# ShawnHymel/ei-keyword-spotting

Measured on AMD Instinct MI355X. Metric: 1s@16kHz clips/sec (MFCC+CNN), higher is better.
Workload: dtype f32

## Files before the change

### ei-keyword-spotting_amd/csrc/kws_fast.hip

```cpp
#include <atomic>

#include "kws_device.h"
#include "kws_fast.h"
#include "kws_bfly_m2k1.h"
#include "kws_fast_maxmin.h"
#if KWS_FAST_WPS >= 3
#define kws_fast_kernel kws_fast_kernel_w3
#define kws_launch_fast kws_launch_fast_w3
#define kws_launch_fast_prof kws_launch_fast_prof_w3
#endif
#include "kws_nn_int8_dev.h"

typedef float v4f __attribute__((ext_vector_type(4)));
#if KWS_FAST_WPS >= 3
#define KWS_OPAQUE3(v) asm volatile("" : "+v"(v))
#define KWS_LANE3(lane) ((int)__builtin_amdgcn_mbcnt_hi(~0u, __builtin_amdgcn_mbcnt_lo(~0u, 0u)))
#define KWS_FAST_SINK (shared + FP.sink_off)
#else
#define KWS_OPAQUE3(v) do { } while (0)
#define KWS_LANE3(lane) (lane)
#define KWS_FAST_SINK (F + FP.sink_off)
#endif
static_assert(KWS_FAST_ZF == KWS_ZF && KWS_FAST_WAVE == KWS_WAVE, "kws_fast.h mirrors kws_device.h");

template <int CTRL> __device__ __forceinline__ float dpp_mov(float v)
{
    return __int_as_float(__builtin_amdgcn_update_dpp(0, __float_as_int(v), CTRL, 0xf, 0xf, true));
}
__device__ __forceinline__ float half_wave_sum(float v)
{
    v += dpp_mov<0xB1>(v);
    v += dpp_mov<0x4E>(v);
    v += dpp_mov<0x141>(v);
    v += dpp_mov<0x140>(v);
    v += __int_as_float(__builtin_amdgcn_ds_swizzle(__float_as_int(v), 0x401F));
    return v;
}
__device__ __forceinline__ float wave_max(float v)
{
    v = fast_max(v, dpp_mov<0xB1>(v));
    v = fast_max(v, dpp_mov<0x4E>(v));
    v = fast_max(v, dpp_mov<0x141>(v));
    v = fast_max(v, dpp_mov<0x140>(v));
    v = fast_max(v, __int_as_float(__builtin_amdgcn_ds_swizzle(__float_as_int(v), 0x401F)));
    return fast_max(v, __shfl_xor(v, 32, KWS_WAVE));
}
__device__ __forceinline__ float wave_sum(float v)
{
    v = half_wave_sum(v);
    return v + __shfl_xor(v, 32, KWS_WAVE);
}
__device__ __forceinline__ float group_sum(float v, int S)
{
    if (S > 1) v += dpp_mov<0xB1>(v);
    if (S > 2) v += dpp_mov<0x4E>(v);
    if (S > 4) v += dpp_mov<0x141>(v);
// ... 746 lines not shown
        WAVE_SYNC();
        if constexpr (SPLIT) {
            _Float16 *const hcol = (_Float16 *)((char *)img + 4 * cb) + cl;
            const bool col_on = lane_on && c < in_cp;
            _Float16 *dst_i = col_on ? hcol + r0 * (2 * fs) : (_Float16 *)sink;
            const int dst_step = col_on ? 2 * fs : 0;
            float sc = c < ncep ? (float)(1 << KWS_SPLIT22_PRE_EXP) : 0.0f;
#pragma unroll
            for (int i = 0; i < CR; ++i) asm volatile("" : "+v"(o[i]));
#pragma unroll
            for (int i = 0; i < CR; ++i) {
                const bool live = CMVN_ROW_LIVE(r0, i);
                _Float16 hi, lo;
                const float d = kws_split22(o[i], sc, &hi, &lo);
                _Float16 *const dst = live ? dst_i : (_Float16 *)sink;
                dst[0] = hi;
                dst[KWS_FAST_PRE_LO / 2] = lo;
                dst_i += dst_step;
                sc = __fmaf_rn(d, 0.0f, sc);
                vacc = live ? __fmaf_rn(gq[i], gq[i], vacc) : vacc;
            }
            vacc = (SAFE > 0 || r0 < nfr) ? __fmaf_rn(sc, 0.0f, vacc) : vacc;
        } else {
#pragma unroll
        for (int i = 0; i < CR; ++i) {
            const int r = r0 + i;
            const bool live = act && r < nfr;
            *(live ? col + r * fs : sink) = o[i];
            if constexpr (DEFER) vacc = live ? __fmaf_rn(gq[i], gq[i], vacc) : vacc;
        }
        }
    }
    WAVE_SYNC();
    return vacc;
#undef CMVN_ROW_LIVE
#undef CMVN_ROW
}

#define KWS_FAST_NPHASE 20
#ifndef KWS_FAST_FULL_PASS
#define KWS_FAST_FULL_PASS (KWS_FAST_WPS >= 3)
#endif
#ifndef KWS_FAST_SOFS
#define KWS_FAST_SOFS (KWS_FAST_WPS >= 3)
#endif
#ifndef KWS_FAST_LATE_ELOG
#define KWS_FAST_LATE_ELOG (KWS_FAST_WPS >= 3)
#endif
#if KWS_FAST_LATE_ELOG
#define KWS_FAST_ELOG(e) (e)
#else
#define KWS_FAST_ELOG(e) fast_log((e) == 0.0f ? FLT_EPSILON : (e))
#endif
#define FPH(i) do { if (PROF) { const long long now_ = clock64(); ph[i] += now_ - tlast; tlast = now_; } } while (0)

template <int NZ, int DG, bool PROF = false, bool FROM_CEP = false, bool NET = true, int QCP = 0, bool MFE = false>
__global__ __launch_bounds__(256 * KWS_FAST_WPS, KWS_FAST_WPS) void kws_fast_kernel(KwsDspPlan P, const KwsFastPlan *__restrict__ FPp, const int16_t *__restrict__ pcm, int n_clips,
                                                          float *__restrict__ scores, float *__restrict__ features,
                                                          int8_t *__restrict__ q_out, float in_scale, int in_zp,
                                                          int *__restrict__ flag_count, int *__restrict__ flag_list,
                                                          long long *__restrict__ prof_out = nullptr, const float *__restrict__ cep = nullptr,
                                                          const KwsNnPlan *__restrict__ QNp = nullptr, const int *__restrict__ sel = nullptr,
                                                          float *__restrict__ tap_logits = nullptr, int feat_in = 0)
{
    static_assert(QCP == 0 || !NET, "the int8 network follows the feature-emitting form");
    static_assert(!MFE || (!NET && QCP == 0 && !FROM_CEP && !PROF), "the MFE form is the spectral prefix: mel energies to HBM");
    const KwsFastPlan &FP = *FPp;
    extern __shared__ __attribute__((aligned(16))) float lds[];
    const int lane = threadIdx.x & (KWS_WAVE - 1), wave = __builtin_amdgcn_readfirstlane((int)(threadIdx.x >> 6));
    if (FROM_CEP && (int)blockIdx.x * (int)(blockDim.x >> 6) >= sel_count(sel, n_clips)) return;
    float *shared = lds;
    float *F = lds + FP.shared_floats + FP.q_floats + wave * FP.wave_floats;
    float *R1 = F + FP.f_floats;
    float *xw = R1, *pw = R1;
    for (int i = threadIdx.x; i < FP.shared_floats; i += blockDim.x) shared[i] = FP.shared_init[i];
    for (int i = lane; i < FP.r1_floats; i += KWS_WAVE) R1[i] = 0.0f;
    constexpr int Q_HEAD = 48 * 256, Q_WB1 = Q_HEAD + ((KWS_HEAD_BYTES + 15) & ~15), Q_WB2 = Q_WB1 + (QCP == 16 ? 4 : 16) * KWS_WAVE * 16,
                  Q_RQ = Q_WB2 + 4 * KWS_WAVE * 16;
    if constexpr (QCP != 0) {
        unsigned char *const qs = (unsigned char *)(lds + FP.shared_floats);
        const KwsNnPlan &QN = *QNp;
        for (int i = threadIdx.x * 4; i < QN.blk[0].out_c * 256; i += blockDim.x * 4) *(int *)(qs + i) = *(const int *)(QN.blk[0].add_lut + i);
        for (int i = threadIdx.x * 4; i < QN.blk[1].out_c * 256; i += blockDim.x * 4) *(int *)(qs + 32 * 256 + i) = *(const int *)(QN.blk[1].add_lut + i);
        (void)nn_head_stage(QN, qs + Q_HEAD);
        nn_mfma_stage_lds<QCP == 0 ? 16 : QCP>(QN, (v4i *)(qs + Q_WB1), (v4i *)(qs + Q_WB2), (int *)(qs + Q_RQ));
    }
    if constexpr (FROM_CEP)
        for (int i = lane; i < FP.wave_floats; i += KWS_WAVE) F[i] = 0.0f;
    __syncthreads();

    const int nfr = P.n_frames, ncep = P.n_cepstral, NF = 8 * DG;
    const int n_tail = (nfr >= KWS_FAST_MEL_CHUNK && (nfr & 7) != 0 && (nfr & 7) <= 2) ? (nfr & 7) : 0;
    const int n_pass = n_tail ? nfr / KWS_FAST_MEL_CHUNK : (nfr + KWS_FAST_MEL_CHUNK - 1) / KWS_FAST_MEL_CHUNK;
    const int fs = FP.fs;
    float *img = F;
    float *elog = F + nfr * fs;
    constexpr int NZ2 = DG > 4 ? KWS_FAST_NZ2 : 1;
    const float *dct_frag = shared + FP.dct_off;
    const int pstride = FP.pstride;
    const int n_waves = blockDim.x >> 6;
    const float pre_cof = P.pre_cof, pscale = kws_fast_pscale(P.inv_fft);
    const int frame_stride = P.frame_stride, n_samples = P.n_samples;
    const float *cnt_tab = shared + FP.cnt_off;
    const int *upd_tab = (const int *)(shared + FP.upd_off);
    const float *ext_tab = FP.ext_off >= 0 ? shared + FP.ext_off : nullptr;
    const float inv_win = FP.inv_win;
    const float *guard_tab = shared + (FROM_CEP ? FP.guard_cep_off : FP.guard_off);
    const int *pad_idx = (const int *)(shared + FP.pad_off);
    const int win_size = P.win_size, prow = nfr + 2 * P.pad;
    const int cr = FP.cr, n_blocks = FP.n_blocks, n_labels = FP.n_labels;
    (void)cr;
    long long ph[KWS_FAST_NPHASE] = { 0 }, tlast = PROF ? clock64() : 0;

    const int clip_stride = gridDim.x * n_waves;
    float *const stash = F + FP.stash_off;
    bool have_stash = false;
    const int n_sel = FROM_CEP ? sel_count(sel, n_clips) : n_clips;
#if KWS_FAST_WPS >= 3
    static_assert(!FROM_CEP, "the forms that start from cepstra are not built for three waves per SIMD");
    int *const tk = FP.tickets;
    int ni = 0;
    for (int ci = blockIdx.x * n_waves + wave; ci < n_sel; ci = ni) {
        int tv = 0;
        if (KWS_LANE3(lane) == 0) tv = __hip_atomic_fetch_add(tk, 1, __ATOMIC_RELAXED, __HIP_MEMORY_SCOPE_AGENT);
        const int clip = FROM_CEP ? sel_clip(sel, ci) : ci;
        const int next_ci = ci;
#else
    for (int ci = blockIdx.x * n_waves + wave; ci < n_sel; ci += clip_stride) {
        const int clip = FROM_CEP ? sel_clip(sel, ci) : ci;
        const int next_ci = ci + clip_stride;
        const int next_clip = ci + clip_stride < n_sel ? ci + clip_stride : -1;
#endif
        int lane_c = KWS_LANE3(lane);
        asm volatile("" : "+v"(lane_c));
        const int fl = lane_c & 7, fg = lane_c >> 3;
        const int nbA = (fl >> 2) + 4 * (fl & 3);
        const float a_c = P.tw[16].x, a_e = P.tw[32].x;
        const cf b1 = to_cf(P.tw[4 * fl]), b2 = to_cf(P.tw[8 * fl]), b3 = to_cf(P.tw[12 * fl]);
#if KWS_FAST_WPS >= 3
        const float *const twl_c = shared + FP.twl_off + 24 * fl, *const twl_s = shared + FP.twl_off + 192 + 16 * fl;
#else
        cf c1[4], c2[4], c3[4];
    #pragma unroll
        for (int a = 0; a < 4; ++a) { c1[a] = to_cf(P.tw[fl + 8 * a]); c2[a] = to_cf(P.tw[2 * (fl + 8 * a)]); c3[a] = to_cf(P.tw[3 * (fl + 8 * a)]); }
        cf stw[8];
    #pragma unroll
        for (int q = 0; q < 8; ++q) {
            const int k = fl + 8 * (q & 3) + 32 * (q >> 2);
            stw[q] = to_cf(P.stw[(k == 0 ? KWS_NC / 2 : k) - 1]);
        }
#endif
        const int xwr = fg * KWS_FAST_XS + 18 * fl;
        const int xrd = fg * KWS_FAST_XS + 2 * fl;
        const int partner = (lane_c & ~7) | ((8 - fl) & 7);
        const int half = lane_c >> 5, t = lane_c & 31;
        const int start1 = FP.tap_start1[lane_c], start2 = FP.tap_start2[lane_c];
        float lvl_sum = 0.0f;
        float w1[NZ], w2[NZ2];
    #pragma unroll
        for (int n = 0; n < NZ; ++n) w1[n] = FP.tap_w1[lane_c * KWS_FAST_NZ_MAX + n];
    #pragma unroll
        for (int n = 0; n < NZ2; ++n) w2[n] = FP.tap_w2[lane_c * KWS_FAST_NZ2 + n];
        int touched_a = 0, touched_b = 0;
        if constexpr (FROM_CEP) {
            const float *src = cep + (size_t)clip * (nfr * ncep);
            const int n_val = nfr * ncep;
            const unsigned inv = (1u << 20) / (unsigned)ncep + 1u;
            const int rr = P.ring_rows, rh = P.ring_head;
            auto ring = [&](int r) { const int t = r + rh; return (rr != 0 && r < rr) ? (t >= rr ? t - rr : t) : r; };
            auto trips = [&](int i_from, int i_to) {
                for (int i0 = i_from + lane; i0 - lane < i_to; i0 += 4 * KWS_WAVE) {
                    float v[4];
                    int dst[4];
// ... 93 lines not shown
                    macc[s] = MFE ? a : fast_log(a);
                }
                float *const d1 = img + (fbase + 4 * half) * fs + t;
#pragma unroll
                for (int s = 0; s < 4; ++s) d1[s * fs] = macc[s];
                if (DG > 4) img[(fbase + sl2) * fs + j2] = macc[4];
                return;
            }
#pragma unroll
            for (int s2 = 0; s2 < 4; s2 += 2) {
                if (s2 >= 2 * pairs) break;
                float xv[2][NZ];
#pragma unroll
                for (int s = 0; s < 2; ++s)
#pragma unroll
                    for (int n = 0; n < NZ; ++n) xv[s][n] = p1[(s2 + s) * pstride + n];
#pragma unroll
                for (int s = 0; s < 2; ++s) {
                    float acc = 0.0f;
#pragma unroll
                    for (int n = 0; n < NZ; ++n) acc = __fmaf_rn(xv[s][n], w1[n], acc);
                    macc[s2 + s] = acc;
                }
            }
            float acc2 = 0.0f;
            if (DG > 4) {
                float xv2[NZ2];
#pragma unroll
                for (int n = 0; n < NZ2; ++n) xv2[n] = p2[n];
#pragma unroll
                for (int n = 0; n < NZ2; ++n) acc2 = __fmaf_rn(xv2[n], w2[n], acc2);
            }
            macc[4] = acc2;
#pragma unroll
            for (int s = 0; s < 5; ++s) {
                const float a = macc[s] == 0.0f ? FLT_EPSILON : macc[s];
                macc[s] = MFE ? a : fast_log(a);
            }
#pragma unroll
            for (int s = 0; s < 4; ++s) {
                const int slot = 4 * half + s;
                if (slot < nfc && t < NF) img[(fbase + slot) * fs + t + (slot == 1 ? adj1 : 0)] = macc[s];
            }
            if (DG > 4 && sl2 < nfc && j2 < NF) img[(fbase + sl2) * fs + j2 + (sl2 == 1 ? adj1 : 0)] = macc[4];
        };
        fast_i2 nxt[2][8];
#if KWS_FAST_SOFS
        if constexpr (SOFS) fetch_at(std::true_type(), sofs0, nxt);
        else
#endif
        fetch(0, nxt);
        int touched = touch(1);
#if KWS_FAST_WPS >= 3
        ni = clip_stride + __builtin_amdgcn_readfirstlane(tv);
        const int next_clip = ni < n_sel ? ni : -1;
#endif
        const bool pair_tail = n_tail == 1 && !have_stash && next_clip >= 0;
        int touched_tail = 0;
        const int16_t *const xnext = pcm + (size_t)max(next_clip, 0) * n_samples;
        if (pair_tail && lane_c < 8) touched_tail = *(const int *)(xnext + (nfr - 1) * frame_stride + 32 * lane_c);
#if KWS_FAST_WPS >= 3
        auto pass_body = [&](int q) {
#else
        for (int q = 0; q < n_pass; ++q) {
#endif
            const int fbase = KWS_FAST_MEL_CHUNK * q;
            const int f = fbase + fg;
            const bool live = f < nfr;
            cf u[4][4];
            {
                cf z[2][8];
#pragma unroll
                for (int blk = 0; blk < 2; ++blk)
#pragma unroll
                    for (int i = 0; i < 8; ++i) z[blk][i] = fast_point(nxt[blk][i], pre_cof);
                if (f == 0 && fl == 0) {
                    fast_i2 v = nxt[0][0];
                    v.y = v.x;
                    v.x = wrap_prev << 16;
                    z[0][0] = fast_point(v, pre_cof);
                }
                fetch(q + 1, nxt);
                asm volatile("" : : "v"(touched));
                touched = touch(q + 2);
                FPH(0);
#pragma unroll
                for (int blk = 0; blk < 2; ++blk) {
                    cf sm[4], df[4];
#pragma unroll
                    for (int i = 0; i < 4; ++i) { sm[i] = cadd(z[blk][2 * i], z[blk][2 * i + 1]); df[i] = csub(z[blk][2 * i], z[blk][2 * i + 1]); }
                    bfly4_unit(sm[0], sm[1], sm[2], sm[3]);
                    bfly4_m2k1(df[0], df[1], df[2], df[3], a_c, a_e);
#pragma unroll
                    for (int i = 0; i < 4; ++i) { z[blk][2 * i] = sm[i]; z[blk][2 * i + 1] = df[i]; }
                }
#pragma unroll
                for (int rnd = 0; rnd < 2; ++rnd) {
#pragma unroll
                    for (int r = 0; r < 8; ++r) *(float2 *)(xw + xwr + 2 * r) = make_float2(z[rnd][r].r, z[rnd][r].i);
                    WAVE_SYNC();
#pragma unroll
                    for (int b = 0; b < 2; ++b)
#pragma unroll
                        for (int a = 0; a < 4; ++a) {
                            const float2 v = *(const float2 *)(xw + xrd + 18 * a + 72 * b);
                            u[a][2 * rnd + b].r = v.x; u[a][2 * rnd + b].i = v.y;
                        }
                    WAVE_SYNC();
                }
            }
#pragma unroll
            for (int b = 0; b < 4; ++b) bfly4(u[0][b], u[1][b], u[2][b], u[3][b], b1, b2, b3);
#pragma unroll
#if KWS_FAST_WPS >= 3
            for (int a = 0; a < 4; ++a) {
                const float4 c12 = *(const float4 *)(twl_c + 6 * a);
                const float2 c3v = *(const float2 *)(twl_c + 6 * a + 4);
                cf t1, t2, t3;
                t1.r = c12.x; t1.i = c12.y; t2.r = c12.z; t2.i = c12.w; t3.r = c3v.x; t3.i = c3v.y;
                bfly4(u[a][0], u[a][1], u[a][2], u[a][3], t1, t2, t3);
            }
            cf stw[8];
#pragma unroll
            for (int q = 0; q < 8; q += 2) {
                const float4 v = *(const float4 *)(twl_s + 2 * q);
                stw[q].r = v.x; stw[q].i = v.y; stw[q + 1].r = v.z; stw[q + 1].i = v.w;
            }
#else
            for (int a = 0; a < 4; ++a) bfly4(u[a][0], u[a][1], u[a][2], u[a][3], c1[a], c2[a], c3[a]);
#endif
            FPH(1);
            {
                float *prow = pw + fg * pstride;
                const bool lane0 = fl == 0;
                float esum = 0.0f;
#pragma unroll
                for (int qq = 0; qq < 8; ++qq) {
// ... 274 lines not shown
            if constexpr (!FROM_CEP) {
                if (silent && FP.sil_off >= 0) {
                    const int half_nf = min(NF / 2, ncep - 1);
                    const float sv = shared[FP.sil_off + min(lane_m + 1, 31)];
                    float *const dst = img + 1 + lane_m;
                    for (unsigned long long mm = smask; mm != 0ull; mm &= mm - 1ull) {
                        const int r = __builtin_ctzll(mm);
                        if (lane_m < half_nf) dst[r * fs] = sv;
                    }
                    n_silent = __popcll(smask);
                    WAVE_SYNC();
                }
            }
            const float mu = wave_sum(on ? x0 : 0.0f) * FP.c0_inv_rows;
            const float d0 = on ? x0 - mu : 0.0f;
            const float sd0 = __builtin_amdgcn_sqrtf(wave_sum(d0 * d0) * FP.c0_inv_rows);
            const float top = wave_max(on ? fabsf(x0) : 0.0f);
            c0_exact = silent || !(FP.c0_factor * sd0 >= __fmaf_rn(FP.c0_rel, top, FP.c0_abs));
        }
        if (c0_exact) {
            constexpr int PS = 260;
            float *pc = R1;
            for (int p = lane_m; p < prow; p += KWS_WAVE) {
                int prw[4];
                float pvv[4];
#pragma unroll
                for (int sft = 0; sft < 4; ++sft) prw[sft] = pad_idx[min(p + sft, prow - 1)];
#pragma unroll
                for (int sft = 0; sft < 4; ++sft) pvv[sft] = img[prw[sft] * fs];
#pragma unroll
                for (int sft = 0; sft < 4; ++sft) pc[sft * PS + p] = pvv[sft];
            }
            WAVE_SYNC();
            const int r = min(lane_m, nfr - 1);
            const float4 *pv = (const float4 *)(pc + (r & 3) * PS + (r & ~3));
            float sum = 0.0f;
            int q = 0;
            const int nq = win_size >> 2;
            for (; q + 4 <= nq; q += 4) {
                float4 v[4];
#pragma unroll
                for (int e = 0; e < 4; ++e) v[e] = pv[q + e];
#pragma unroll
                for (int e = 0; e < 4; ++e) { sum += v[e].x; sum += v[e].y; sum += v[e].z; sum += v[e].w; }
            }
            for (; q < nq; ++q) { const float4 v = pv[q]; sum += v.x; sum += v.y; sum += v.z; sum += v.w; }
            {
                const float4 v = pv[q];
                const int rem = win_size & 3;
                if (rem > 0) sum += v.x;
                if (rem > 1) sum += v.y;
                if (rem > 2) sum += v.z;
            }
            if (lane_m < nfr) elog[lane_m] = __fdiv_rn(sum, (float)win_size);
            WAVE_SYNC();
        }
        if (PROF) { const long long now_ = clock64(); ph[19] += now_ - tlast; }
        if constexpr (QCP != 0) {
            const int z1 = (int)((unsigned)(QNp->blk[0].in_zp & 0xff) * 0x01010101u);
            for (int i = lane_m; i < KWS_A1_ROWS * (QCP / 4); i += KWS_WAVE) ((int *)act1)[i] = z1;
            WAVE_SYNC();
        }
        float gV = 0.0f;
        if constexpr (!MFE) {
          if (feats_given) gV = FP.v_net_feat;
          else {
            float level = FROM_CEP ? 0.0f : wave_sum(lvl_sum) * FP.lvl_inv, abs_scale = 1.0f;
            if (!FROM_CEP && n_silent > 0) {
                const float live = (float)(nfr - n_silent), rows = (float)nfr;
                level = live > 0.0f ? fmaxf(__fmaf_rn(level, rows, (float)n_silent * fast_log(FLT_EPSILON)), 0.0f) / live : 0.0f;
                abs_scale = __builtin_amdgcn_sqrtf(live / rows);
                level *= abs_scale;
            }
#if KWS_FAST_WPS >= 3
            constexpr bool TWO_COPIES = !(NZ == 8 && DG == 5);
            if (TWO_COPIES && nfr >= 3 * 13 + 9) vlane = fast_cmvn<13, 16, true, true, 9>(img, cnt_tab, upd_tab, fs, inv_win, guard_tab, level, abs_scale, silent, FP.sys_t2, piv_row, elog, c0_exact, lane_m, nfr, ncep, ext_tab, csink, FP.blk[0].in_cp);
            else vlane = fast_cmvn<13, 16, true, true>(img, cnt_tab, upd_tab, fs, inv_win, guard_tab, level, abs_scale, silent, FP.sys_t2, piv_row, elog, c0_exact, lane_m, nfr, ncep, ext_tab, csink, FP.blk[0].in_cp);
#else
            if (cr == 13) vlane = fast_cmvn<13, 16, QCP == 0>(img, cnt_tab, upd_tab, fs, inv_win, guard_tab, level, abs_scale, silent, FP.sys_t2, piv_row, elog, c0_exact, lane_m, nfr, ncep, ext_tab, csink);
            else vlane = fast_cmvn<17, 20, QCP == 0>(img, cnt_tab, upd_tab, fs, inv_win, guard_tab, level, abs_scale, silent, FP.sys_t2, piv_row, elog, c0_exact, lane_m, nfr, ncep, ext_tab, csink);
#endif
            gV = __int_as_float(__builtin_amdgcn_readfirstlane(__float_as_int(wave_sum(vlane) + FP.v_net)));
          }
        }
        if constexpr (!NET) {
            if (!MFE && !(gV * fmaxf(FP.g_c1 * 0.0625f, FP.g_c2) <= 1.0f)) {
                if (lane == 0) flag_list[atomicAdd(flag_count, 1)] = clip;
            }
        }
        if constexpr (!NET) {
            const unsigned inv = (1u << 20) / (unsigned)ncep + 1u;
            const int q_pad = QCP != 0 ? QNp->blk[0].pad_left : 0;
            for (int i = lane; i < nfr * ncep; i += KWS_WAVE) {
                const int r = (int)(((unsigned)i * inv) >> 20), c = i - r * ncep;
                const float o = img[r * fs + c];
                if (fout) fout[i] = o;
                if (QCP != 0 || qclip) {
                    const int8_t qb = quantize_feature(o, in_scale, in_zp);
                    if (qclip) qclip[i] = qb;
                    if constexpr (QCP != 0) act1[(r + q_pad) * QCP + c] = qb;
                }
            }
            WAVE_SYNC();
        }
        FPH(5);
        if constexpr (QCP != 0) {
            const KwsNnPlan &QN = *QNp;
            int8_t *const act2 = (int8_t *)F;
            int *const vec = (int *)(F + KWS_A2_ROWS * 8);
            const int z2 = (int)((unsigned)(QN.blk[1].in_zp & 0xff) * 0x01010101u);
            for (int i = lane; i < KWS_A2_ROWS * 8; i += KWS_WAVE) ((int *)act2)[i] = z2;
            WAVE_SYNC();
            unsigned char *const qs = (unsigned char *)(lds + FP.shared_floats);
            const NnMfmaLds<QCP> qctx = nn_mfma_lds_ctx<QCP>(QN, (const v4i *)(qs + Q_WB1), (const v4i *)(qs + Q_WB2), (const int *)(qs + Q_RQ), lane);
            const NnHeadTab q_head = nn_head_tab(qs + Q_HEAD);
            const NnTaps no_taps = { nullptr, 0, nullptr, nullptr, nullptr, nullptr };
            __builtin_amdgcn_s_setprio(1);
            nn_mfma_clip<QCP>(qctx, QN, q_head, act1, act2, vec, (const int8_t *)qs, (const int8_t *)qs + 32 * 256, lane, clip, scores, no_taps);
            __builtin_amdgcn_s_setprio(0);
            WAVE_SYNC();
        }
        if constexpr (FROM_CEP) asm volatile("" : : "v"(touched_a), "v"(touched_b));
        if constexpr (!NET) continue;
        else {

        float *cur = F, *oth = R1;
#if KWS_FAST_WPS >= 3
        int lane_n = KWS_LANE3(lane);
        asm volatile("" : "+v"(lane_n));
        int ws_off = FP.sink_off + lane_n;
        asm volatile("" : "+v"(ws_off));
        float *const wsink = shared + ws_off;
#else
        float *const wsink = KWS_FAST_SINK + lane;
        int lane_n = lane;
        asm volatile("" : "+v"(lane_n));
#endif
        for (int b = 0; b < n_blocks; ++b) {
            const KwsFastBlock &k = FP.blk[b];
            int lane_b = lane_n;
            KWS_OPAQUE3(lane_b);
            const bool last = b + 1 == n_blocks;
            const int o_stride = last ? k.out_c : FP.blk[b + 1].in_stride;
            const int o_cp = last ? k.out_c : FP.blk[b + 1].in_cp;
            const bool pooled = k.pool > 1 || k.pool_stride > 1;
            float *stage = pooled ? cur : oth;
            const int sstride = pooled ? k.stage_stride : o_stride;
            long long t_loop = 0, t_pre = 0, *tl = (PROF && b == 0) ? &t_loop : nullptr, *tp = (PROF && b == 0) ? &t_pre : nullptr;
            if (k.dw) {
                fast_dwconv(k, cur, oth, shared, lane_b, o_stride, o_cp);
                WAVE_SYNC();
                float *tmp = cur; cur = oth; oth = tmp;
                if (PROF && b > 0) { const long long now_ = clock64(); ph[12 + b] += now_ - tlast; }
                FPH(6 + (b > 0));
                continue;
            }
            float cscale = 1.0f;
            if (k.hconv) {
                const int zo = FP.zero_off;
                const bool bgl = k.h_b_off < 0;
                const bool pre = KWS_FAST_WPS >= 3 && b == 0;
                if (bgl && k.n_tiles == 1 && k.m_tiles == 1 && k.h_ks <= 8) cscale = fast_conv_small_h<1>(k, cur, stage, sstride, shared, zo, lane_b, wsink, pre);
                else
                switch ((k.m_tiles > 2 ? 4 : k.m_tiles) * 4 + k.n_tiles) {
                case 4 * 4 + 2: cscale = bgl ? fast_conv_tiles_h<4, 2, true>(k, cur, stage, sstride, shared, zo, lane_b, wsink, pre) : fast_conv_tiles_h<4, 2, false, (DG > 4)>(k, cur, stage, sstride, shared, zo, lane_b, wsink, pre); break;
                case 4 * 4 + 1: cscale = bgl ? fast_conv_tiles_h<4, 1, true>(k, cur, stage, sstride, shared, zo, lane_b, wsink, pre) : fast_conv_tiles_h<4, 1, false>(k, cur, stage, sstride, shared, zo, lane_b, wsink, pre); break;
                case 2 * 4 + 2: cscale = bgl ? fast_conv_tiles_h<2, 2, true>(k, cur, stage, sstride, shared, zo, lane_b, wsink, pre) : fast_conv_tiles_h<2, 2, false>(k, cur, stage, sstride, shared, zo, lane_b, wsink, pre); break;
                case 2 * 4 + 1: cscale = bgl ? fast_conv_tiles_h<2, 1, true>(k, cur, stage, sstride, shared, zo, lane_b, wsink, pre) : fast_conv_tiles_h<2, 1, false>(k, cur, stage, sstride, shared, zo, lane_b, wsink, pre); break;
                case 1 * 4 + 2: cscale = bgl ? fast_conv_tiles_h<1, 2, true>(k, cur, stage, sstride, shared, zo, lane_b, wsink, pre) : fast_conv_tiles_h<1, 2, false>(k, cur, stage, sstride, shared, zo, lane_b, wsink, pre); break;
                default: cscale = bgl ? fast_conv_tiles_h<1, 1, true>(k, cur, stage, sstride, shared, zo, lane_b, wsink, pre) : fast_conv_tiles_h<1, 1, false>(k, cur, stage, sstride, shared, zo, lane_b, wsink, pre); break;
                }
            } else
            switch (k.m_tiles * 4 + k.n_tiles) {
            case 4 * 4 + 2: fast_conv_tiles<4, 2>(k, cur, stage, sstride, shared, lane_b, wsink, tl, tp); break;
            case 4 * 4 + 1: fast_conv_tiles<4, 1>(k, cur, stage, sstride, shared, lane_b, wsink); break;
            case 3 * 4 + 2: fast_conv_tiles<3, 2>(k, cur, stage, sstride, shared, lane_b, wsink, tl, tp); break;
            case 3 * 4 + 1: fast_conv_tiles<3, 1>(k, cur, stage, sstride, shared, lane_b, wsink); break;
            case 2 * 4 + 2: fast_conv_tiles<2, 2>(k, cur, stage, sstride, shared, lane_b, wsink); break;
            case 2 * 4 + 1: fast_conv_tiles<2, 1>(k, cur, stage, sstride, shared, lane_b, wsink); break;
            case 1 * 4 + 2: fast_conv_tiles<1, 2>(k, cur, stage, sstride, shared, lane_b, wsink); break;
            default: fast_conv_tiles<1, 1>(k, cur, stage, sstride, shared, lane_b, wsink); break;
            }
            WAVE_SYNC();
            if (PROF && b == 0 && t_loop != 0) { ph[9] += t_loop - t_pre; ph[10] += clock64() - t_loop; ph[11] += t_pre - tlast; }
            if (k.fpool) fast_pool_finish(k, stage, oth, shared, lane_b, o_stride, o_cp, cscale);
            else fast_pool(k, stage, oth, lane_b, o_stride, o_cp, pooled);
            WAVE_SYNC();
            float *tmp = cur; cur = oth; oth = tmp;
            if (PROF && b > 0) { const long long now_ = clock64(); ph[12 + b] += now_ - tlast; }
            FPH(6 + (b > 0));
        }
        {
            const int fc_in = FP.fc_in, fc_out = FP.fc_out;
            const int sh = fc_out > 1 ? 32 - __builtin_clz(fc_out - 1) : 0;
            const int S = KWS_WAVE >> sh, unit = lane_n >> (6 - sh), sl = lane_n & (S - 1), uc = min(unit, fc_out - 1);
            const float *wfc = shared + FP.fc_w_off + uc * fc_in;
            float tot = 0.0f, tot1 = 0.0f;
            int i = sl;
            for (; i + S < fc_in; i += 2 * S) { tot = __fmaf_rn(cur[i], wfc[i], tot); tot1 = __fmaf_rn(cur[i + S], wfc[i + S], tot1); }
            if (i < fc_in) tot = __fmaf_rn(cur[i], wfc[i], tot);
            tot = group_sum(tot + tot1, S) + shared[FP.fc_b_off + uc];
            tot = fast_clamp_u(tot, FP.fc_min, FP.fc_max);
            const bool on = unit < fc_out;
            if (tap_logits && on && sl == 0) tap_logits[(size_t)clip * n_labels + unit] = tot;
            const float mx = wave_max(on ? tot : -FLT_MAX);
            const float e = expf((tot - mx) * FP.beta);
            const float sum = wave_sum(on && sl == 0 ? e : 0.0f);
            const float pr = e / sum;
            if (on && sl == 0) scores[(size_t)clip * n_labels + unit] = pr;
            const float pq = wave_max(on && sl == 0 ? pr * (1.0f - pr) : 0.0f);
            if (!(gV * fmaxf(FP.g_c1 * pq * pq, FP.g_c2) <= 1.0f)) {
                if (lane_n == 0) flag_list[atomicAdd(flag_count, 1)] = clip;
            }
        }
        WAVE_SYNC();
        FPH(8);
        }
    }
#if KWS_FAST_WPS >= 3
    if (lane == 0) {
        const int gone = __hip_atomic_fetch_add(FP.tickets + 1, 1, __ATOMIC_RELAXED, __HIP_MEMORY_SCOPE_AGENT);
        if (gone == (int)(gridDim.x * (blockDim.x >> 6)) - 1) {
            __hip_atomic_store(FP.tickets, 0, __ATOMIC_RELAXED, __HIP_MEMORY_SCOPE_AGENT);
            __hip_atomic_store(FP.tickets + 1, 0, __ATOMIC_RELAXED, __HIP_MEMORY_SCOPE_AGENT);
        }
    }
#endif
    if (PROF && blockIdx.x == 0 && threadIdx.x == 0 && prof_out)
        for (int i = 0; i < KWS_FAST_NPHASE; ++i) prof_out[i] = ph[i];
}

#ifndef KWS_FAST_NO_LAUNCHERS
#if KWS_FAST_WPS < 3
int kws_launch_fast_w3(const KwsDspPlan &P, const KwsFastPlan &FP, const KwsFastPlan *d_plan, const int16_t *pcm, int n_clips, float *scores, float *features,
                       int8_t *q_out, float in_scale, int in_zp, int *flag_count, int *flag_list, int n_cu, hipStream_t stream, const KwsNnPlan *d_nn, float *tap_logits);
int kws_launch_fast_prof_w3(const KwsDspPlan &P, const KwsFastPlan &FP, const KwsFastPlan *d_plan, const int16_t *pcm, int n_clips, float *scores,
                            int *flag_count, int *flag_list, int n_cu, long long *prof_out, hipStream_t stream);
#endif
template <int NZ, int DG, bool PROF, bool FROM_CEP = false, bool NET = true, int QCP = 0, bool MFE = false>
static int launch_fast_t(const KwsDspPlan &P, const KwsFastPlan &FP, const KwsFastPlan *d_plan, const int16_t *pcm, int n_clips, float *scores,
                         float *features, int8_t *q_out, float in_scale, int in_zp, int *flag_count, int *flag_list, int n_cu,
                         long long *prof_out, hipStream_t stream, const float *cep = nullptr, const KwsNnPlan *d_nn = nullptr, const int *sel = nullptr,
                         float *tap_logits = nullptr, int feat_in = 0)
{
    const size_t smem = ((size_t)FP.shared_floats + FP.q_floats + (size_t)FP.n_waves * FP.wave_floats) * sizeof(float);
    static std::atomic<unsigned long long> attr_done{ 0 };
    int dev = 0;
    if (hipGetDevice(&dev) != hipSuccess) return (int)hipGetLastError();
    const unsigned long long bit = 1ull << (dev & 63);
    if (!(attr_done.load(std::memory_order_acquire) & bit)) {
        if (hipFuncSetAttribute((const void *)kws_fast_kernel<NZ, DG, PROF, FROM_CEP, NET, QCP, MFE>, hipFuncAttributeMaxDynamicSharedMemorySize, 160 * 1024) != hipSuccess)
            return (int)hipGetLastError();
        attr_done.fetch_or(bit, std::memory_order_release);
    }
    const int per_wg = FP.n_waves;
    int grid = (n_clips + per_wg - 1) / per_wg;
    if (grid > n_cu) grid = n_cu;
#if KWS_FAST_WPS >= 3
    if (!FP.tickets) return (int)hipErrorInvalidValue;
#endif
    hipLaunchKernelGGL((kws_fast_kernel<NZ, DG, PROF, FROM_CEP, NET, QCP, MFE>), dim3(grid), dim3(KWS_WAVE * FP.n_waves), smem, stream, P, d_plan, pcm, n_clips, scores,
                       features, q_out, in_scale, in_zp, flag_count, flag_list, prof_out, cep, d_nn, sel, tap_logits, feat_in);
    return (int)hipGetLastError();
}

int kws_launch_fast(const KwsDspPlan &P, const KwsFastPlan &FP, const KwsFastPlan *d_plan, const int16_t *pcm, int n_clips, float *scores,
                    float *features, int8_t *q_out, float in_scale, int in_zp, int *flag_count, int *flag_list, int n_cu, hipStream_t stream,
                    const KwsNnPlan *d_nn, float *tap_logits)
{
    (void)hipGetLastError();
    if (n_clips <= 0) return 0;
#define KWS_FAST_ARGS P, FP, d_plan, pcm, n_clips, scores, features, q_out, in_scale, in_zp, flag_count, flag_list, n_cu, nullptr, stream
#define KWS_FAST_NARGS KWS_FAST_ARGS, nullptr, nullptr, nullptr, tap_logits
#if KWS_FAST_WPS >= 3
    if (FP.wps != KWS_FAST_WPS || FP.qnet || FP.mfe || !FP.fuse || !FP.presplit) return (int)hipErrorInvalidValue;
#define KWS_FAST_PLAIN(...) ((int)hipErrorInvalidValue)
#else
// ... 77 lines not shown
```

### ei-keyword-spotting_amd/csrc/kws_fast_plan.cpp

```cpp
#include "kws_internal.h"
#include "kws_bfly_m2k1.h"
#include <atomic>
#include <cstdlib>

static const int kLdsBytes = 160 * 1024;

static int round_up(int v, int m) { return (v + m - 1) / m * m; }

static uint16_t f32_to_f16(float f)
{
    uint32_t u;
    memcpy(&u, &f, sizeof u);
    const uint32_t sign = (u >> 16) & 0x8000u;
    u &= 0x7fffffffu;
    if (u >= 0x47800000u) return (uint16_t)(sign | (u > 0x7f800000u ? 0x7e00u : 0x7c00u));
    if (u < 0x38800000u) {
        if (u < 0x33000000u) return (uint16_t)sign;
        const int shift = 126 - (int)(u >> 23);
        const uint32_t m = (u & 0x7fffffu) | 0x800000u;
        uint32_t h = m >> shift;
        const uint32_t rem = m & ((1u << shift) - 1u), half = 1u << (shift - 1);
        if (rem > half || (rem == half && (h & 1u))) h++;
        return (uint16_t)(sign | h);
    }
    uint32_t h = ((u - 0x38000000u) >> 13);
    const uint32_t rem = u & 0x1fffu;
    if (rem > 0x1000u || (rem == 0x1000u && (h & 1u))) h++;
    return (uint16_t)(sign | h);
}
static float f16_to_f32(uint16_t h)
{
    const uint32_t sign = (uint32_t)(h & 0x8000u) << 16, e = (h >> 10) & 0x1fu, m = h & 0x3ffu;
    float f;
    if (e == 0) f = ldexpf((float)m, -24);
    else if (e == 31) f = m ? NAN : INFINITY;
    else f = ldexpf((float)(m | 0x400u), (int)e - 25);
    uint32_t u;
    memcpy(&u, &f, sizeof u);
    u |= sign;
    memcpy(&f, &u, sizeof f);
    return f;
}

static const float kGuardK = 4.5f, kGuardLin = 1.1f, kGuardScoreTol = 1.0e-4f, kGuardLogitCap = 0.1f;
static const float kAbs0 = 4.5e-7f, kAlpha0 = 0.6e-7f, kAlphaDct = 1.7e-7f, kAlphaStale = 2.0e-8f, kKappa = 0.3e-6f, kKappa0 = 1.0e-7f, kKappaStale = 0.14e-6f, kKappaSilent = 0.9e-6f, kFloorCep = 3.0e-7f, kRhoDev = 3.0e-7f,
                   kC0Share = 0.05f, kSysRatio = 3.0e-3f;
static const float kAlphaDct40[21] = { 0.f, 6.4e-7f, 2.5e-7f, 1.8e-7f, 1.4e-7f, 1.5e-7f, 1.1e-7f, 0.94e-7f, 0.87e-7f, 0.90e-7f, 1.73e-7f, 0.90e-7f, 0.80e-7f, 0.77e-7f, 0.78e-7f,
                                       1.2e-7f, 0.82e-7f, 0.74e-7f, 0.73e-7f, 0.96e-7f, 2.26e-7f };
static const float kAlphaDct32[13] = { 0.f, 4.1e-7f, 1.8e-7f, 1.3e-7f, 1.22e-7f, 0.80e-7f, 0.86e-7f, 0.66e-7f, 1.46e-7f, 0.60e-7f, 0.78e-7f, 0.52e-7f, 1.03e-7f };
static float alpha_dct(int NF, int c)
{
    if (NF == 40 && c >= 1 && c <= 20) return kAlphaDct40[c];
    if (NF == 32 && c >= 1 && c <= 12) return kAlphaDct32[c];
    return kAlphaDct;
// ... 289 lines not shown
static void fast_wave_floats(const kws_handle *h, KwsFastPlan &F, int need_f, int need_r1)
{
    const int nfr = h->dsp.n_frames;
    if (F.wps >= 3) {
        F.f_floats = round_up(std::max(nfr * F.fs + nfr, need_f), 4) + 48;
    } else {
        F.f_floats = round_up(std::max(nfr * F.fs + nfr, need_f), 4) + KWS_FAST_WAVE + 48;
        F.sink_off = F.f_floats - KWS_FAST_WAVE - 48;
    }
    F.stash_off = F.f_floats - 48;
    F.r1_floats = round_up(std::max(std::max(KWS_FAST_MEL_CHUNK * KWS_FAST_XS, KWS_FAST_MEL_CHUNK * F.pstride), need_r1), 4);
    F.wave_floats = F.f_floats + F.r1_floats;
}

static EI_IMPULSE_ERROR finish_fast_plan(kws_handle *h, KwsFastPlan &F, std::vector<float> &shared, int need_f, int need_r1)
{
    const KwsDspPlan &P = h->dsp;
    const int nfr = P.n_frames;
    std::vector<int> pmap;
    h_pad_map(nfr, P.pad, pmap);
    for (int r = 0; r + 1 < nfr; r++) {
        const int packed = (pmap[r] * F.fs) | ((pmap[r + P.win_size] * F.fs) << 16);
        memcpy(&shared[(size_t)F.upd_off + r], &packed, sizeof(int));
    }
    if (F.ext_off >= 0)
        for (int g = 0; g < KWS_FAST_WAVE / F.cg; g++)
            for (int n = 0; n < KWS_FAST_CMVN_EXT; n++) {
                int row;
                float *slot = &shared[(size_t)F.ext_off + (size_t)g * (1 + 2 * KWS_FAST_CMVN_EXT) + 1 + 2 * n];
                memcpy(&row, slot, sizeof(int));
                row *= F.fs;
                memcpy(slot, &row, sizeof(int));
            }
    while (shared.size() & 3) shared.push_back(0.0f);
    if (F.wps >= 3) {
        F.sink_off = (int)shared.size();
        shared.insert(shared.end(), KWS_FAST_WAVE + KWS_FAST_PRE_LO / 4, 0.0f);
    }
    F.shared_floats = (int)shared.size();
    fast_wave_floats(h, F, need_f, need_r1);
    const int avail = kLdsBytes / 4 - F.shared_floats - F.q_floats;
    F.n_waves = std::min(4 * F.wps, avail / F.wave_floats);
    if (const char *ev = KWS_DEV_ENV("KWS_DEV_FAST_WAVES")) F.n_waves = std::max(1, std::min(F.n_waves, atoi(ev)));
    if (KWS_DEV_ENV("KWS_DEV_FAST_REPORT"))
        fprintf(stderr, "fast plan: shared %d B + q %d B + %d waves x %d B (F %d + R1 %d) of %d; built for %d waves per SIMD\n", F.shared_floats * 4, F.q_floats * 4, F.n_waves,
                F.wave_floats * 4, F.f_floats * 4, F.r1_floats * 4, kLdsBytes, F.wps);
    if (F.n_waves < 4 && !KWS_DEV_ENV("KWS_DEV_FAST_WAVES")) return fail(KWS_ERROR_UNSUPPORTED_MODEL, "fast mode: %d B shared + %d B per wave does not leave four waves per workgroup",
                                   F.shared_floats * 4, F.wave_floats * 4);
    EI_IMPULSE_ERROR e = h->upload(shared, &F.shared_init);
    if (e) return e;
    F.tickets = nullptr;
    if (F.wps >= 3) {
        const int *dev = nullptr;
        if ((e = h->upload(std::vector<int>(4, 0), &dev))) return e;
        F.tickets = const_cast<int *>(dev);
    }
    std::vector<KwsFastPlan> one(1, F);
    return h->upload(one, &F == &h->fast_fused ? &h->d_fast_fused : &F == &h->fast_fused_cep ? &h->d_fast_fused_cep : &F == &h->fast_q ? &h->d_fast_q : &h->d_fast_plain);
}

static EI_IMPULSE_ERROR build_fast_plain(kws_handle *h)
{
    KwsFastPlan &F = h->fast_plain;
    memset(&F, 0, sizeof(F));
    F.wps = 2;
    std::vector<float> shared;
    EI_IMPULSE_ERROR e = build_fast_dsp(h, F, shared);
    if (e) return e;
    F.fs = h->dsp.n_filters + 4;
    F.fuse = 0;
    F.n_labels = (int)h->model.labels.size();
    return finish_fast_plan(h, F, shared, 0, 0);
}

static EI_IMPULSE_ERROR build_fast_q(kws_handle *h)
{
    KwsFastPlan &F = h->fast_q;
    memset(&F, 0, sizeof(F));
    F.wps = 2;
    if (h->is_float) return fail(KWS_ERROR_UNSUPPORTED_MODEL, "fast mode: the fused int8 network needs an int8 graph");
    if (h->fast_plain.mfe) return fail(KWS_ERROR_UNSUPPORTED_MODEL, "fast mode: the MFE block's normalisation sits between the front end and the network (not fused)");
    if (!kws_nn_uses_mfma(h->nn)) return fail(KWS_ERROR_UNSUPPORTED_MODEL, "fast mode: the int8 graph is outside the two-block matrix-core shape; it keeps its own kernel");
    const int qcp = h->nn.blk[0].in_cpad == 16 ? 16 : 64;
    if ((qcp == 16) != (h->dsp.n_filters == 32))
        return fail(KWS_ERROR_UNSUPPORTED_MODEL, "fast mode: %d-byte activation rows with %d mel filters is not an instantiated pairing", qcp, h->dsp.n_filters);
    std::vector<float> shared;
    EI_IMPULSE_ERROR e = build_fast_dsp(h, F, shared);
    if (e) return e;
    F.fs = h->dsp.n_filters + 4;
    F.fuse = 0;
    F.n_labels = (int)h->model.labels.size();
    F.qnet = qcp;
    F.q_floats = (int)((kws_fast_qnet_bytes(qcp) + 15) / 16 * 4);
    if (!h->d_nn) {
        std::vector<KwsNnPlan> one(1, h->nn);
        if ((e = h->upload(one, &h->d_nn))) return e;
    }
    return finish_fast_plan(h, F, shared, 24 * 8 + 96, 72 * qcp / 4);
}

static EI_IMPULSE_ERROR build_fast_fused(kws_handle *h, int wps, KwsFastPlan &F)
{
    memset(&F, 0, sizeof(F));
    F.wps = wps;
    if (!h->is_float) return fail(KWS_ERROR_UNSUPPORTED_MODEL, "fast mode: the fused network is float32 (int8 graphs keep their exact kernels)");
    if (h->fast_plain.mfe) return fail(KWS_ERROR_UNSUPPORTED_MODEL, "fast mode: the MFE block's normalisation sits between the front end and the network (not fused)");
    const KwsNnPlanF32 &N = h->nnf;
// ... 193 lines not shown
```

Baseline: 58.16 million.

## Shard the dynamic clip ticket counter across eight cache-line-separated counters

Replaces the single global atomic ticket counter used for dynamic clip scheduling in the three-waves-per-SIMD kernel with eight shards, each on its own padded line. A block draws from its home shard, and once that shard is exhausted it steals from the other shards in turn. The aim is to reduce atomic contention on one address, at the cost of extra atomics near the end of the clip range and a more complex reset. It also adds profiling counters and makes win_size opaque in the elog division.

```diff
diff --git a/ei-keyword-spotting_amd/csrc/kws_fast.hip b/ei-keyword-spotting_amd/csrc/kws_fast.hip
--- a/ei-keyword-spotting_amd/csrc/kws_fast.hip
+++ b/ei-keyword-spotting_amd/csrc/kws_fast.hip
@@ -2,6 +2,7 @@
 
 #include "kws_device.h"
 #include "kws_fast.h"
+#include "kws_fast_ticket.h"
 #include "kws_bfly_m2k1.h"
 #include "kws_fast_maxmin.h"
 #if KWS_FAST_WPS >= 3
@@ -854,6 +855,7 @@
 #else
 #define KWS_FAST_ELOG(e) fast_log((e) == 0.0f ? FLT_EPSILON : (e))
 #endif
+#define KWS_FAST_PROF_BLOCK(b) (KWS_FAST_WPS >= 3 ? (b) > 0 && (b) < 4 : (b) > 0)
 #define FPH(i) do { if (PROF) { const long long now_ = clock64(); ph[i] += now_ - tlast; tlast = now_; } } while (0)
 
 template <int NZ, int DG, bool PROF = false, bool FROM_CEP = false, bool NET = true, int QCP = 0, bool MFE = false>
@@ -920,7 +922,7 @@
     const int n_sel = FROM_CEP ? sel_count(sel, n_clips) : n_clips;
 #if KWS_FAST_WPS >= 3
     static_assert(!FROM_CEP, "the forms that start from cepstra are not built for three waves per SIMD");
-    int *const tk = FP.tickets;
+    int *const tk = FP.tickets + kws_fast_ticket_head(kws_fast_ticket_home((int)blockIdx.x));
     int ni = 0;
     for (int ci = blockIdx.x * n_waves + wave; ci < n_sel; ci = ni) {
         int tv = 0;
@@ -1120,7 +1122,8 @@
         fetch(0, nxt);
         int touched = touch(1);
 #if KWS_FAST_WPS >= 3
-        ni = clip_stride + __builtin_amdgcn_readfirstlane(tv);
+        const int tk_home = kws_fast_ticket_home((int)blockIdx.x);
+        ni = kws_fast_ticket_clip(clip_stride, tk_home, __builtin_amdgcn_readfirstlane(tv));
         const int next_clip = ni < n_sel ? ni : -1;
 #endif
         const bool pair_tail = n_tail == 1 && !have_stash && next_clip >= 0;
@@ -1135,6 +1138,7 @@
             const int fbase = KWS_FAST_MEL_CHUNK * q;
             const int f = fbase + fg;
             const bool live = f < nfr;
+            const long long ptop = PROF && KWS_FAST_WPS >= 3 ? clock64() : 0;
             cf u[4][4];
             {
                 cf z[2][8];
@@ -1151,6 +1155,7 @@
                 fetch(q + 1, nxt);
                 asm volatile("" : : "v"(touched));
                 touched = touch(q + 2);
+                if (PROF && KWS_FAST_WPS >= 3) { ph[q == 0 ? 18 : 16] += clock64() - ptop; ph[17] += q == 0; }
                 FPH(0);
 #pragma unroll
                 for (int blk = 0; blk < 2; ++blk) {
@@ -1531,7 +1536,13 @@
                 if (rem > 1) sum += v.y;
                 if (rem > 2) sum += v.z;
             }
+#if KWS_FAST_WPS >= 3
+            int win_here = win_size;
+            asm volatile("" : "+s"(win_here));
+            if (lane_m < nfr) elog[lane_m] = __fdiv_rn(sum, (float)win_here);
+#else
             if (lane_m < nfr) elog[lane_m] = __fdiv_rn(sum, (float)win_size);
+#endif
             WAVE_SYNC();
         }
         if (PROF) { const long long now_ = clock64(); ph[19] += now_ - tlast; }
@@ -1630,7 +1641,7 @@
                 fast_dwconv(k, cur, oth, shared, lane_b, o_stride, o_cp);
                 WAVE_SYNC();
                 float *tmp = cur; cur = oth; oth = tmp;
-                if (PROF && b > 0) { const long long now_ = clock64(); ph[12 + b] += now_ - tlast; }
+                if (PROF && KWS_FAST_PROF_BLOCK(b)) { const long long now_ = clock64(); ph[12 + b] += now_ - tlast; }
                 FPH(6 + (b > 0));
                 continue;
             }
@@ -1666,7 +1677,7 @@
             else fast_pool(k, stage, oth, lane_b, o_stride, o_cp, pooled);
             WAVE_SYNC();
             float *tmp = cur; cur = oth; oth = tmp;
-            if (PROF && b > 0) { const long long now_ = clock64(); ph[12 + b] += now_ - tlast; }
+            if (PROF && KWS_FAST_PROF_BLOCK(b)) { const long long now_ = clock64(); ph[12 + b] += now_ - tlast; }
             FPH(6 + (b > 0));
         }
         {
@@ -1695,13 +1706,22 @@
         WAVE_SYNC();
         FPH(8);
         }
+#if KWS_FAST_WPS >= 3
+        if (ni >= n_sel) {
+            ni = kws_fast_ticket_walk(clip_stride, n_sel, kws_fast_ticket_home((int)blockIdx.x), [&](int s) {
+                int v = 0;
+                if (lane == 0) v = __hip_atomic_fetch_add(FP.tickets + kws_fast_ticket_head(s), 1, __ATOMIC_RELAXED, __HIP_MEMORY_SCOPE_AGENT);
+                return __builtin_amdgcn_readfirstlane(v);
+            });
+        }
+#endif
     }
 #if KWS_FAST_WPS >= 3
     if (lane == 0) {
-        const int gone = __hip_atomic_fetch_add(FP.tickets + 1, 1, __ATOMIC_RELAXED, __HIP_MEMORY_SCOPE_AGENT);
+        const int gone = __hip_atomic_fetch_add(FP.tickets + kws_fast_ticket_gone(), 1, __ATOMIC_RELAXED, __HIP_MEMORY_SCOPE_AGENT);
         if (gone == (int)(gridDim.x * (blockDim.x >> 6)) - 1) {
-            __hip_atomic_store(FP.tickets, 0, __ATOMIC_RELAXED, __HIP_MEMORY_SCOPE_AGENT);
-            __hip_atomic_store(FP.tickets + 1, 0, __ATOMIC_RELAXED, __HIP_MEMORY_SCOPE_AGENT);
+            for (int s = 0; s < KWS_FAST_TICKET_SHARDS; ++s) __hip_atomic_store(FP.tickets + kws_fast_ticket_head(s), 0, __ATOMIC_RELAXED, __HIP_MEMORY_SCOPE_AGENT);
+            __hip_atomic_store(FP.tickets + kws_fast_ticket_gone(), 0, __ATOMIC_RELAXED, __HIP_MEMORY_SCOPE_AGENT);
         }
     }
 #endif
diff --git a/ei-keyword-spotting_amd/csrc/kws_fast_plan.cpp b/ei-keyword-spotting_amd/csrc/kws_fast_plan.cpp
--- a/ei-keyword-spotting_amd/csrc/kws_fast_plan.cpp
+++ b/ei-keyword-spotting_amd/csrc/kws_fast_plan.cpp
@@ -1,5 +1,6 @@
 #include "kws_internal.h"
 #include "kws_bfly_m2k1.h"
+#include "kws_fast_ticket.h"
 #include <atomic>
 #include <cstdlib>
 
@@ -395,7 +396,7 @@
     F.tickets = nullptr;
     if (F.wps >= 3) {
         const int *dev = nullptr;
-        if ((e = h->upload(std::vector<int>(4, 0), &dev))) return e;
+        if ((e = h->upload(std::vector<int>(KWS_FAST_TICKET_WORDS, 0), &dev))) return e;
         F.tickets = const_cast<int *>(dev);
     }
     std::vector<KwsFastPlan> one(1, F);
diff --git a/ei-keyword-spotting_amd/csrc/kws_fast_ticket.h b/ei-keyword-spotting_amd/csrc/kws_fast_ticket.h
--- /dev/null
+++ b/ei-keyword-spotting_amd/csrc/kws_fast_ticket.h
@@ -0,0 +1,31 @@
+#pragma once
+
+#if defined(__HIPCC__) || defined(__CUDACC__)
+#define KWS_TICKET_HD __host__ __device__
+#else
+#define KWS_TICKET_HD
+#endif
+
+#ifndef KWS_FAST_TICKET_SHARDS
+#define KWS_FAST_TICKET_SHARDS 8
+#endif
+#define KWS_FAST_TICKET_LINE 32
+#define KWS_FAST_TICKET_WORDS ((KWS_FAST_TICKET_SHARDS + 1) * KWS_FAST_TICKET_LINE)
+
+KWS_TICKET_HD static inline int kws_fast_ticket_home(int block) { return block % KWS_FAST_TICKET_SHARDS; }
+KWS_TICKET_HD static inline int kws_fast_ticket_head(int shard) { return shard * KWS_FAST_TICKET_LINE; }
+KWS_TICKET_HD static inline int kws_fast_ticket_gone(void) { return KWS_FAST_TICKET_SHARDS * KWS_FAST_TICKET_LINE; }
+KWS_TICKET_HD static inline int kws_fast_ticket_clip(int stride, int shard, int t) { return stride + KWS_FAST_TICKET_SHARDS * t + shard; }
+
+template <class Draw>
+KWS_TICKET_HD static inline int kws_fast_ticket_walk(int stride, int n_sel, int home, Draw draw)
+{
+    int c = n_sel;
+#pragma unroll 1
+    for (int k = 1; k < KWS_FAST_TICKET_SHARDS; ++k) {
+        const int s = home + k < KWS_FAST_TICKET_SHARDS ? home + k : home + k - KWS_FAST_TICKET_SHARDS;
+        c = kws_fast_ticket_clip(stride, s, draw(s));
+        if (c < n_sel) break;
+    }
+    return c;
+}
```

Result: faster. 59.22 million, median of 6 (+1.8%).
